# khiner/MeshEditor

Hardware: AMD Instinct MI355X
Metric: eigenpairs/sec (K/M assembly + 50-mode solve, 100k-tet mesh) (higher is better)
Workload: dtype f64; 1 GPU; cube_s100k: Kuhn mesh 105456 tets / 446631 DOF, NumModes=50 NumFemModes=65, P=10 excitation points, one mesh per GPU; eigenpairs_per_mesh=65, kept_modes_per_mesh=50, parallelism=mesh-per-gpu x1

## Files before the change

mesheditor_amd/csrc/lab/mh_lab.hip:

```cpp
#include "../mh_common.h"
#include "modalhip_lab.h"

#include <algorithm>

void mh_elementwise_apply(mh_context *ctx, const mh_system *sys, double sigma, const double *x, double *y, uint32_t w);

namespace {
constexpr int TB = 256;
__global__ void k_lab_ref_to_panel(const double *__restrict__ x, const uint32_t *__restrict__ perm, uint32_t nnodes, uint32_t width, double *__restrict__ panel) {
    const size_t i = size_t(blockIdx.x) * blockDim.x + threadIdx.x;
    if (i >= size_t(nnodes) * 3 * width) return;
    const uint32_t c = uint32_t(i % width), comp = uint32_t((i / width) % 3), node = uint32_t(i / (size_t(3) * width));
    panel[i] = x[size_t(c) * (size_t(3) * nnodes) + size_t(3) * perm[node] + comp];
}
__global__ void k_lab_panel_to_ref(const double *__restrict__ panel, const uint32_t *__restrict__ perm, uint32_t nnodes, uint32_t width, double *__restrict__ y) {
    const size_t i = size_t(blockIdx.x) * blockDim.x + threadIdx.x;
    if (i >= size_t(nnodes) * 3 * width) return;
    const uint32_t c = uint32_t(i % width), comp = uint32_t((i / width) % 3), node = uint32_t(i / (size_t(3) * width));
    y[size_t(c) * (size_t(3) * nnodes) + size_t(3) * perm[node] + comp] = panel[i];
}
}

namespace {
typedef float f4_stream __attribute__((ext_vector_type(4)));
// ... 417 lines not shown
            const std::vector<uint32_t> h = ps.nodes.to_host();
            for (size_t i = 0; i < h.size(); ++i) nodes[i] = node_ref[h[i]];
        }
        if (weight && ps.n_patches) ps.weight.download(weight, ps.n_patches);
        if (inv64 && ps.n_patches) ps.inv64.download(inv64, ps.inv64.count);
        if (cluster_row && ps.n_clusters) {
            const std::vector<uint32_t> h = ps.cluster_row.to_host();
            for (size_t i = 0; i < h.size(); ++i) cluster_row[i] = 3 * node_ref[h[i] / 3] + h[i] % 3;
        }
        if (cluster_ptr && ps.n_clusters) std::copy(ps.h_cluster_ptr.begin(), ps.h_cluster_ptr.end(), cluster_ptr);
        if (cinv64 && ps.n_clusters) ps.cinv64.download(cinv64, ps.cinv64.count);
        return MH_OK;
    } catch (const std::exception &e) { return mh_guard(ctx, e); }
}

int mhl_context_potrf_inverse(mh_context *ctx, uint32_t w, const double *a, const double *dscale, double *l, double *linv, int *info2) {
    if (!ctx || !a || !dscale || !l || !linv || !info2 || w < 1 || w > 128) return MH_EINVAL;
    try {
        HIP_CHECK(hipSetDevice(ctx->device));
        MhSharedPhase not_during_a_factorisation(ctx->device);
        DevArray<double> da(ctx, size_t(w) * w), dd(ctx, w), dl(ctx, size_t(w) * w);
        DevArray<int> info(ctx, 2);
        da.upload(a, size_t(w) * w);
        dd.upload(dscale, w);
        mh_potrf_small_inverse(ctx, da, w, info, dd, dl);
        da.download(l, size_t(w) * w);
        dl.download(linv, size_t(w) * w);
        info.download(info2, 2);
        return MH_OK;
    } catch (const std::exception &e) { return mh_guard(ctx, e); }
}

int mhl_context_spd_inverse(mh_context *ctx, uint32_t w, const double *a, double *out, uint32_t reps, double *avg_ms) {
    if (!ctx || !a || !out || w < 1 || w > 128) return MH_EINVAL;
    try {
        HIP_CHECK(hipSetDevice(ctx->device));
        MhSharedPhase not_during_a_factorisation(ctx->device);
        DevArray<double> da(ctx, size_t(w) * w), dout(ctx, size_t(w) * w);
        DevArray<int> info(ctx, 1);
        info.zero();
        da.upload(a, size_t(w) * w);
        hipEvent_t e0, e1;
        HIP_CHECK(hipEventCreate(&e0));
        HIP_CHECK(hipEventCreate(&e1));
        float total = 0;
        for (uint32_t r = 0; r < std::max(1u, reps); ++r) {
            HIP_CHECK(hipEventRecord(e0, ctx->stream));
            mh_spd_inverse_small(ctx, da, w, w, dout, w, info);
            HIP_CHECK(hipEventRecord(e1, ctx->stream));
            HIP_CHECK(hipEventSynchronize(e1));
            float ms = 0;
            HIP_CHECK(hipEventElapsedTime(&ms, e0, e1));
            total += ms;
        }
        (void)hipEventDestroy(e0);
        (void)hipEventDestroy(e1);
        dout.download(out, size_t(w) * w);
        int hinfo = 0;
        info.download(&hinfo, 1);
        if (avg_ms) *avg_ms = total / std::max(1u, reps);
        return hinfo ? MH_EFACTOR : MH_OK;
    } catch (const std::exception &e) { return mh_guard(ctx, e); }
}

int mhl_context_small_gemm(mh_context *ctx, int ta, int tb, uint32_t M, uint32_t N, uint32_t K, double alpha, const double *a, uint32_t lda, const double *b, uint32_t ldb, double beta,
                           double *c, uint32_t ldc, uint32_t reps, double *avg_ms) {
    if (!ctx || !a || !b || !c || !M || !N || !K || lda < (ta ? K : M) || ldb < (tb ? N : K) || ldc < M) return MH_EINVAL;
    try {
        HIP_CHECK(hipSetDevice(ctx->device));
        MhSharedPhase not_during_a_factorisation(ctx->device);
        const size_t na = size_t(lda) * (ta ? M : K), nb = size_t(ldb) * (tb ? K : N), nc = size_t(ldc) * N;
        DevArray<double> da(ctx, na), db(ctx, nb), dc(ctx, nc), work(ctx, nc);
        da.upload(a, na);
        db.upload(b, nb);
        dc.upload(c, nc);
        hipEvent_t e0, e1;
        HIP_CHECK(hipEventCreate(&e0));
        HIP_CHECK(hipEventCreate(&e1));
        float total = 0;
        for (uint32_t r = 0; r < std::max(1u, reps); ++r) {
            HIP_CHECK(hipMemcpyAsync(work, dc, nc * sizeof(double), hipMemcpyDeviceToDevice, ctx->stream));
// ... 93 lines not shown
```

mesheditor_amd/csrc/mh_common.h:

```cpp
#pragma once
#include "../../include/modalhip.h"

#include <hip/hip_runtime.h>
#include <rocblas/rocblas.h>
#include <rocsolver/rocsolver.h>

#include <algorithm>
#include <cstdarg>
#include <cstdio>
#include <cstdlib>
#include <cstring>
#include <iterator>
#include <limits>
#include <map>
#include <mutex>
#include <stdexcept>
#include <string>
#include <vector>

struct MhError : std::runtime_error {
    int code;
    MhError(int c, const std::string &m) : std::runtime_error(m), code(c) {}
};

// ... 461 lines not shown
uint32_t mh_shift_invert_panel(mh_system *sys, double sigma, const double *b, double *x, uint32_t w, double rel_tol, uint32_t max_iters, double *worst_rel);
struct MhCycleShape {
    int deg2{2}, deg1{5}, gamma{3};
    double ratio{8.0}, ratio1{0.0};
};
void mh_cycle_shape(const mh_system *sys, uint32_t w, MhCycleShape *shape);
double mh_coarse_lift(const mh_system *sys);
void mh_precondition_panel(mh_system *sys, double sigma, int precision, const double *r, double *z, uint32_t w);
uint32_t mh_graph_aggregates(const std::vector<uint32_t> &row_ptr, const std::vector<uint32_t> &col, uint32_t n, uint32_t target, uint32_t max_order, std::vector<uint32_t> &agg_of);
void mh_select_patches(mh_system *sys, float threshold);
void mh_build_patch_inverses(mh_context *ctx, const BsrLevel &lvl, PatchSet &ps);
template<typename T>
void mh_apply_patches(mh_context *ctx, const PatchSet &ps, const T *in, const T *minus, uint32_t w, T coef, T *d, T *x, double *z, uint32_t wz, T *scratch);
void mh_gram(mh_context *ctx, size_t n, const double *x, uint32_t wa, const double *y, uint32_t wb, double *g, uint32_t ld, uint32_t ldy = 0, const uint32_t *ymap = nullptr);
void mh_combine(mh_context *ctx, size_t n, const double *x, uint32_t wx, const double *w, uint32_t ww, const double *p, uint32_t wp, const double *ct, uint32_t nc,
                double *out1, uint32_t n1, double *out2, bool accumulate = false, uint32_t ldx = 0, const uint32_t *xmap = nullptr, uint32_t ld1 = 0,
                const uint32_t *omap = nullptr, uint32_t col_begin = 0, uint32_t col_count = 0);
bool mh_tridiag_lowest_wide(mh_context *ctx, const double *d, const double *e, uint32_t m, uint32_t k, double *w, double *z, uint32_t ldz, double *work, int *info2,
                            double *quality_host);
void mh_apply_q(mh_context *ctx, const double *a, const double *tau, uint32_t m, double *z, uint32_t ldz, uint32_t ncols);
bool mh_tridiag_lowest(mh_context *ctx, const double *d, const double *e, uint32_t m, uint32_t k, double *w, double *z, uint32_t ldz, double *ufac,
                       double *quality, double *lam_scratch);
struct MhRrTrace {
    enum Reduction { GIVEN_IDENTITY = 0, MEASURED_IDENTITY = 1, SERIES = 2, CHOLESKY = 3 };
    enum Solver { SYEVD = 0, SMALL_PARTIAL = 1, SMALL_STEDC = 2, WIDE_PARTIAL = 3, WIDE_STEDC_ORMTR = 4 };
    int reduction{-1};
    double defect{-1};
    int solver{-1};
    double quality{std::numeric_limits<double>::quiet_NaN()};
};
int mh_rr_solve(mh_context *ctx, double *gA, double *gM, uint32_t m, double *evals, double *ework, DevArray<int> &info, uint32_t nwant = 0, bool gm_is_identity = false,
                std::vector<double> *host_evals = nullptr);
void mh_spd_inverse_small(mh_context *ctx, const double *a, uint32_t lda, uint32_t w, double *out, uint32_t ldo, int *info);
void mh_potrf(mh_context *ctx, double *a, uint32_t ld, uint32_t w, int *info);
void mh_potrf_small(mh_context *ctx, double *a, uint32_t w, int *info);
void mh_potrf_small_inverse(mh_context *ctx, double *a, uint32_t w, int *info, const double *dscale, double *linv);
bool mh_sytrd_gave_up(mh_context *ctx);
void mh_sytrd_wide(mh_context *ctx, double *a, uint32_t m, double *d, double *e, double *tau);
void mh_sytrd_small(mh_context *ctx, double *a, uint32_t m, double *d, double *e, double *tau, int variant = -1);
void mh_small_gemm(mh_context *ctx, bool ta, bool tb, uint32_t M, uint32_t N, uint32_t K, double alpha, const double *a, uint32_t lda, const double *b, uint32_t ldb, double beta, double *c,
                   uint32_t ldc);
void mh_short_product(mh_context *ctx, size_t n, const double *a, uint32_t m, const double *ct, uint32_t nc, double *out, double *partial, uint32_t slices);
void mh_pack_stacked(mh_context *ctx, const double *c1, uint32_t r1, const double *c2, uint32_t r2, uint32_t cols, double scale, double *ct);
void mh_pack_coefficients(mh_context *ctx, const double *c1, uint32_t n1, const double *c2, uint32_t n2, uint32_t m, uint32_t ld, double *ct);
void mh_spmm_mapped(mh_context *ctx, const BsrLevel &lvl, const double *vals9, const double *x, double *y, const double *mscal, double *y2, uint32_t w, uint32_t ldy,
                    uint32_t wreal, const uint32_t *omap, const double *res_theta = nullptr, double *res_out = nullptr, double *res_partial = nullptr,
                    const double *res_dinv = nullptr);
bool mh_spmm_f32_cheb_step(mh_context *ctx, const BsrLevel &lvl, const float *d_in, float *d_out, float *r, float *x, const float *dinv, float c1, float c2,
                           uint32_t w);
void mh_spmm_f32(mh_context *ctx, const BsrLevel &lvl, const float *x, float *y, uint32_t w);
void mh_spmm_mixed(mh_context *ctx, const BsrLevel &lvl, const float *x, double *y, uint32_t w);
const uint32_t *mh_identity_map(mh_context *ctx);
void mh_spmm(mh_context *ctx, const BsrLevel &lvl, const double *vals9, const double *x, double *y, const double *mscal, double *y2, uint32_t w);
```

mesheditor_amd/csrc/mh_dense.hip:

```cpp
#include "mh_common.h"

#include <optional>

#include <map>

struct PerDeviceOnce {
    static constexpr int MaxDevices = 64;
    std::once_flag flag[MaxDevices];
    template<typename F> void run(int device, F &&f) { std::call_once(flag[device >= 0 && device < MaxDevices ? device : 0], std::forward<F>(f)); }
};

static bool mh_test_own_gemm() {
    static const bool on = getenv("MH_TEST") && strstr(getenv("MH_TEST"), "own_gemm");
    return on;
}
namespace {
constexpr int KC = 32;

typedef double double4_t __attribute__((ext_vector_type(4)));

__host__ __device__ inline int pad_pitch(int w) {
    int p = ((w + 15) / 16) * 16;
    if ((p % 32) != 16) p += 16;
    return p;
// ... 2121 lines not shown
    const double *ap = A + (a_ok ? ia : 0) * sai + k_lane * sak, *bp = B + (b_ok ? jb : 0) * sbj + k_lane * sbk;
    double4_t acc = {0, 0, 0, 0};
    int k = 0;
    for (; k + 32 <= K; k += 32) {
        double af[8], bf[8];
#pragma unroll
        for (int u = 0; u < 8; ++u) af[u] = ap[(k + 4 * u) * sak], bf[u] = bp[(k + 4 * u) * sbk];
#pragma unroll
        for (int u = 0; u < 8; ++u) acc = __builtin_amdgcn_mfma_f64_16x16x4f64(a_ok ? af[u] : 0.0, b_ok ? bf[u] : 0.0, acc, 0, 0, 0);
    }
    for (; k < K; k += 4) {
        const bool k_ok = k + k_lane < K;
        const double av = a_ok && k_ok ? ap[k * sak] : 0.0, bv = b_ok && k_ok ? bp[k * sbk] : 0.0;
        acc = __builtin_amdgcn_mfma_f64_16x16x4f64(av, bv, acc, 0, 0, 0);
    }
    if (!b_ok) return;
#pragma unroll
    for (int reg = 0; reg < 4; ++reg) {
        const int row = i0 + k_lane + 4 * reg;
        if (row >= M) continue;
        double *c = C + size_t(jb) * ldc + row;
        *c = beta == 0.0 ? alpha * acc[reg] : alpha * acc[reg] + beta * *c;
    }
}
}

void mh_small_gemm(mh_context *ctx, bool ta, bool tb, uint32_t M, uint32_t N, uint32_t K, double alpha, const double *a, uint32_t lda, const double *b, uint32_t ldb, double beta, double *c,
                   uint32_t ldc) {
    if (!M || !N) return;
    const dim3 grid(div_up(M, 32), div_up(N, 32));
    k_small_gemm<<<grid, 256, 0, ctx->stream>>>(int(M), int(N), int(K), alpha, a, ta ? long(lda) : 1L, ta ? 1L : long(lda), b, tb ? long(ldb) : 1L, tb ? 1L : long(ldb), beta, c, int(ldc));
    KERNEL_CHECK();
}
```

mesheditor_amd/csrc/mh_eigs.hip:

```cpp
#include "mh_common.h"

#include <algorithm>
#include <cmath>
#include <memory>
#include <condition_variable>
#include <mutex>
#include <numeric>
#include <optional>
#include <type_traits>

__global__ void k_shift_values(const double *kval, const double *mval, size_t nblocks, double sigma, double *aval);
__global__ void k_diag_inverse(const uint32_t *row_ptr, const uint32_t *col, const double *aval, uint32_t nnodes, double *dinv);
__global__ void k_coarse_matrix(const uint32_t *row_ptr, const uint32_t *col, const double *aval, const double *tmat, const uint32_t *agg_of, const uint32_t *agg_ptr,
                                const uint32_t *agg_nodes, uint32_t nagg, double *a0);
__global__ void k_fix_coarse_diag(double *a0, uint32_t n0, double rel);

namespace {
constexpr int TB = 256;

std::mutex g_solve_mutex;
struct Switches {
    bool verbose = getenv("MH_VERBOSE") != nullptr;
    bool fp32_prec = !(getenv("MH_PRECOND_FP64") && atoi(getenv("MH_PRECOND_FP64")) != 0);
    int deg2 = 0, deg1 = 0, gamma = 0;
// ... 658 lines not shown
    HIP_CHECK(hipMemcpyAsync(saved.get(), gA, size_t(m) * m * sizeof(double), hipMemcpyDeviceToDevice, ctx->stream));
    mh_sytrd_wide(ctx, gA, m, evals, ework, tau);
    int gave_up = 0;
    HIP_CHECK(hipMemcpyAsync(&gave_up, ctx->sytrd_flag, sizeof(int), hipMemcpyDeviceToHost, ctx->stream));
    HIP_CHECK(hipStreamSynchronize(ctx->stream));
    if (sytrd_gave_up(ctx, gave_up, gA, saved, m)) return std::nullopt;
    if (nwant && nwant < m && nwant <= 256 && !switches().no_tridiag_wide) {
        DevArray<double> work(ctx, size_t(5) * nwant * m + size_t(2) * nwant * nwant + 8), lam(ctx, nwant);
        double quality = 1.0;
        if (mh_tridiag_lowest_wide(ctx, evals, ework, m, nwant, lam, z, m, work, info, &quality)) {
            if (switches().verbose) fprintf(stderr, "[rr] tridiagonal m %u lowest %u (wide): residual / ||T|| %.2e\n", m, nwant, quality);
            if (ctx->rr_trace) ctx->rr_trace->quality = quality;
            if (accept_partial(ctx, quality, evals, lam, nwant)) {
                if (ctx->rr_trace) ctx->rr_trace->solver = MhRrTrace::WIDE_PARTIAL;
                mh_apply_q(ctx, gA, tau, m, z, m, nwant);
                rr_selfcheck(ctx, saved.get(), m, z, m, evals, nwant);
                HIP_CHECK(hipMemcpyAsync(gA, z.get(), size_t(m) * nwant * sizeof(double), hipMemcpyDeviceToDevice, ctx->stream));
                HIP_CHECK(hipStreamSynchronize(ctx->stream));
                return 0;
            }
        }
    }
    ROCBLAS_CHECK(rocsolver_dstedc(ctx->blas, rocblas_evect_tridiagonal, m, evals, ework, z, m, info));
    if (const int hinfo = host_info(info)) return hinfo;
    ROCBLAS_CHECK(rocsolver_dormtr(ctx->blas, rocblas_side_left, rocblas_fill_lower, rocblas_operation_none, m, m, gA, m, tau, z, m));
    if (ctx->rr_trace) ctx->rr_trace->solver = MhRrTrace::WIDE_STEDC_ORMTR;
    HIP_CHECK(hipMemcpyAsync(gA, z.get(), size_t(m) * m * sizeof(double), hipMemcpyDeviceToDevice, ctx->stream));
    HIP_CHECK(hipStreamSynchronize(ctx->stream));
    return 0;
}

}

int mh_rr_solve(mh_context *ctx, double *gA, double *gM, uint32_t m, double *evals, double *ework, DevArray<int> &info, uint32_t nwant, bool gm_is_identity,
                std::vector<double> *host_evals) {
    const double one = 1, zero = 0;
    k_symmetrize_lower<<<grid1(size_t(m) * m), TB, 0, ctx->stream>>>(gA, m, m);
    KERNEL_CHECK();
    bool identity = gm_is_identity, series = false;
    if (!identity) {
        static_assert(sizeof(unsigned long long) == sizeof(double), "defect word");
        unsigned long long *defect = reinterpret_cast<unsigned long long *>(ework);
        HIP_CHECK(hipMemsetAsync(defect, 0, sizeof(unsigned long long), ctx->stream));
        k_identity_defect<<<grid1(size_t(m) * m), TB, 0, ctx->stream>>>(gM, m, defect);
        KERNEL_CHECK();
        unsigned long long bits = 0;
        HIP_CHECK(hipMemcpyAsync(&bits, defect, sizeof(bits), hipMemcpyDeviceToHost, ctx->stream));
        HIP_CHECK(hipStreamSynchronize(ctx->stream));
        double d;
        memcpy(&d, &bits, sizeof(d));
        identity = d < 1e-11;
        if (switches().verbose) fprintf(stderr, "[rr] m %u identity defect %.2e\n", m, d);
        series = !identity && d < 1e-7;
        if (ctx->rr_trace) ctx->rr_trace->defect = d;
    }
    if (ctx->rr_trace) ctx->rr_trace->reduction = gm_is_identity ? MhRrTrace::GIVEN_IDENTITY : identity ? MhRrTrace::MEASURED_IDENTITY : series ? MhRrTrace::SERIES : MhRrTrace::CHOLESKY;
    DevArray<double> sroot, stmp;
    if (series) {
        sroot.reset(ctx, size_t(m) * m);
        stmp.reset(ctx, size_t(m) * m * 2);
        double *e = stmp.get(), *e2 = stmp.get() + size_t(m) * m;
        k_defect_matrix<<<grid1(size_t(m) * m), TB, 0, ctx->stream>>>(gM, m, e);
        KERNEL_CHECK();
        small_dgemm(ctx, rocblas_operation_none, rocblas_operation_none, m, m, m, &one, e, m, e, m, &zero, e2, m);
        k_inverse_sqrt_series<<<grid1(size_t(m) * m), TB, 0, ctx->stream>>>(e, e2, m, sroot);
        KERNEL_CHECK();
// ... 315 lines not shown
    {
        const uint32_t nb = 128;
        DevArray<double> &cblk = sys->coarse_ws[0], &rblk = sys->coarse_ws[1], &pnext = sys->coarse_ws[4];
        DevArray<double> *pinv2[2] = {&sys->coarse_ws[2], &sys->coarse_ws[3]};
        cblk.reset(ctx, n0 * nb);
        rblk.reset(ctx, n0 * nb);
        pinv2[0]->reset(ctx, size_t(nb) * nb);
        pinv2[1]->reset(ctx, size_t(nb) * nb);
        pnext.reset(ctx, size_t(nb) * nb);
        info.zero();
        const bool side = ctx->aux_stream_ready();
        struct StreamGuard {
            mh_context *c;
            hipStream_t s;
            bool swapped{false};
            ~StreamGuard() {
                if (c->stream != s) {
                    c->stream = s;
                    if (swapped) std::swap(c->blas, c->blas_aux);
                    (void)hipStreamSynchronize(c->aux_stream);
                    if (c->aux2_stream) (void)hipStreamSynchronize(c->aux2_stream);
                }
            }
        } guard{ctx, main_stream};
        hipEvent_t forked = nullptr;
        if (side) {
            HIP_CHECK(hipEventCreateWithFlags(&forked, hipEventDisableTiming));
            HIP_CHECK(hipEventRecord(forked, main_stream));
            HIP_CHECK(hipStreamWaitEvent(ctx->aux_stream, forked, 0));
            ctx->stream = ctx->aux_stream;
            std::swap(ctx->blas, ctx->blas_aux);
            guard.swapped = true;
        }
        const size_t steps_total = div_up(n0, size_t(nb));
        const bool ahead = side && ctx->aux2_stream_ready(2 * steps_total);
        hipEvent_t *ev_piv = ctx->ahead_ev.data(), *ev_inv = ctx->ahead_ev.data() + steps_total;
        const double one = 1, zero = 0, mone = -1;
        const rocblas_int ld = rocblas_int(n0);
        double *a = sys->a0.get();
        uint32_t step = 0;
        for (size_t k0 = 0; k0 < n0; k0 += nb, ++step) {
            const rocblas_int w = rocblas_int(std::min<size_t>(nb, n0 - k0));
            double *pinv = pinv2[step & 1]->get();
            if (step == 0 || !ahead) mh_spd_inverse_small(ctx, a + k0 * n0 + k0, uint32_t(n0), uint32_t(w), pinv, uint32_t(w), info);
            else HIP_CHECK(hipStreamWaitEvent(ctx->stream, ev_inv[step], 0));
            HIP_CHECK(hipMemcpyAsync(cblk, a + k0 * n0, n0 * size_t(w) * sizeof(double), hipMemcpyDeviceToDevice, ctx->stream));
            ROCBLAS_CHECK(rocblas_dgemm(ctx->blas, rocblas_operation_none, rocblas_operation_none, w, ld, w, &one, pinv, w, a + k0, ld, &zero, rblk, w));
            const size_t k1 = k0 + nb;
            if (ahead && k1 < n0) {
                const uint32_t wn = uint32_t(std::min<size_t>(nb, n0 - k1));
                HIP_CHECK(hipMemcpy2DAsync(pnext.get(), size_t(wn) * sizeof(double), a + k1 * n0 + k1, n0 * sizeof(double), size_t(wn) * sizeof(double), wn, hipMemcpyDeviceToDevice, ctx->stream));
                mh_small_gemm(ctx, false, false, wn, wn, uint32_t(w), -1.0, cblk.get() + k1, uint32_t(n0), rblk.get() + k1 * size_t(w), uint32_t(w), 1.0, pnext.get(), wn);
                HIP_CHECK(hipEventRecord(ev_piv[step], ctx->stream));
                HIP_CHECK(hipStreamWaitEvent(ctx->aux2_stream, ev_piv[step], 0));
                hipStream_t elimination = ctx->stream;
                ctx->stream = ctx->aux2_stream;
                try {
                    mh_spd_inverse_small(ctx, pnext.get(), wn, wn, pinv2[(step + 1) & 1]->get(), wn, info);
                } catch (...) {
                    ctx->stream = elimination;
                    throw;
                }
                ctx->stream = elimination;
                HIP_CHECK(hipEventRecord(ev_inv[step + 1], ctx->aux2_stream));
            }
            ROCBLAS_CHECK(rocblas_dgemm(ctx->blas, rocblas_operation_none, rocblas_operation_none, ld, ld, w, &mone, cblk, ld, rblk, w, &one, a, ld));
            HIP_CHECK(hipMemcpy2DAsync(a + k0, n0 * sizeof(double), rblk.get(), size_t(w) * sizeof(double), size_t(w) * sizeof(double), n0, hipMemcpyDeviceToDevice, ctx->stream));
            ROCBLAS_CHECK(rocblas_dgemm(ctx->blas, rocblas_operation_none, rocblas_operation_none, ld, w, w, &mone, cblk, ld, pinv, w, &zero, a + k0 * n0, ld));
            HIP_CHECK(hipMemcpy2DAsync(a + k0 * n0 + k0, n0 * sizeof(double), pinv, size_t(w) * sizeof(double), size_t(w) * sizeof(double), size_t(w), hipMemcpyDeviceToDevice, ctx->stream));
        }
        k_symmetrize_lower<<<grid1(n0 * n0), TB, 0, ctx->stream>>>(sys->a0, uint32_t(n0), uint32_t(n0));
        KERNEL_CHECK();
        if (side) {
            ctx->stream = main_stream;
            std::swap(ctx->blas, ctx->blas_aux);
        }
        if (!sys->coarse_done) HIP_CHECK(hipEventCreateWithFlags(&sys->coarse_done, hipEventDisableTiming));
        HIP_CHECK(hipEventRecord(sys->coarse_done, side ? ctx->aux_stream : main_stream));
        sys->coarse_pending = true;
        smoother_setup();
        if (side) (void)hipEventDestroy(forked);
    }
    sys->sigma_built = sigma;
    sys->hierarchy_ready = true;
    if (!defer) {
        mh_finish_hierarchy(sys);
        HIP_CHECK(hipStreamSynchronize(ctx->stream));
    }
}

namespace {
__global__ void k_last_columns_to_panel(const double *__restrict__ z, size_t n, uint32_t ncols, const double *__restrict__ scale, double *__restrict__ x) {
    const size_t i = size_t(blockIdx.x) * blockDim.x + threadIdx.x;
    if (i >= n * ncols) return;
    const uint32_t j = uint32_t(i % ncols);
    x[i] = scale[j] * z[(n - 1 - j) * n + i / ncols];
}

void dense_eigs(mh_system *sys, uint32_t nev, double sigma, double *eigenvalues, bool inverse = false) {
    mh_context *ctx = sys->ctx;
    const size_t n = size_t(3) * sys->n_nodes;
    auto &lvl = sys->L2;
    DevArray<double> a(ctx, n * n), m(ctx, n * n), d(ctx, n), e(ctx, n);
    DevArray<int> info(ctx, 1);
    a.zero();
// ... 971 lines not shown
```

mesheditor_amd/csrc/mh_patch.hip:

```cpp
#include "mh_common.h"

namespace {
constexpr int TB = 256;
struct PerDeviceOnce {
    std::mutex m;
    bool done[64] = {};
    template<typename F> void run(int device, F &&f) {
        std::lock_guard<std::mutex> l(m);
        if (!done[unsigned(device) % 64]) f(), done[unsigned(device) % 64] = true;
    }
};

__global__ void k_element_quality(const double *__restrict__ pts, const uint32_t *__restrict__ elem_ref, uint32_t stride, uint32_t nt, float *__restrict__ q, float threshold,
                                  uint32_t *__restrict__ summary) {
    const uint32_t el_raw = blockIdx.x * blockDim.x + threadIdx.x;
    const bool valid = el_raw < nt;
    const uint32_t el = valid ? el_raw : nt - 1;
    double v[4][3];
    for (int a = 0; a < 4; ++a)
        for (int d = 0; d < 3; ++d) v[a][d] = pts[3 * size_t(elem_ref[size_t(el) * stride + a]) + d];
    const double bx = v[1][0] - v[0][0], by = v[1][1] - v[0][1], bz = v[1][2] - v[0][2];
    const double cx = v[2][0] - v[0][0], cy = v[2][1] - v[0][1], cz = v[2][2] - v[0][2];
    const double dx = v[3][0] - v[0][0], dy = v[3][1] - v[0][1], dz = v[3][2] - v[0][2];
    const double vol = fabs(dx * (by * cz - cy * bz) + dy * (bz * cx - cz * bx) + dz * (bx * cy - cx * by)) / 6;
// ... 227 lines not shown
        if (r >= N) continue;
#pragma unroll
        for (int j = 0; j < 4; ++j) {
            const uint32_t cc = col0 + tx * 4 + j;
            if (cc < w) y[size_t(r0 + r) * w + cc] = acc[i][j];
        }
    }
}

template<typename T>
__global__ void k_cluster_scatter(const T *__restrict__ y, uint32_t w, const uint32_t *__restrict__ crow, uint32_t nrows, T coef, T *__restrict__ d, T *__restrict__ x, double *__restrict__ z,
                                  uint32_t wz, int slices) {
    const size_t i = size_t(blockIdx.x) * blockDim.x + threadIdx.x;
    if (i >= size_t(nrows) * w) return;
    const uint32_t c = uint32_t(i % w);
    const size_t row = crow[i / w];
    T sum = 0;
    for (int q = 0; q < slices; ++q) sum += y[size_t(q) * nrows * w + i];
    const T s = coef * sum;
    if (d) d[row * w + c] += s;
    if (x) x[row * w + c] += s;
    if (z && c < wz) z[row * wz + c] += double(s);
}

__global__ void k_f64_to_f32(const double *__restrict__ in, float *__restrict__ out, size_t count) {
    const size_t i = size_t(blockIdx.x) * blockDim.x + threadIdx.x;
    if (i < count) out[i] = float(in[i]);
}
__global__ void k_copy_block(const double *__restrict__ in, uint32_t ldi, double *__restrict__ out, uint32_t ldo, uint32_t rows, uint32_t cols) {
    const size_t i = size_t(blockIdx.x) * blockDim.x + threadIdx.x;
    if (i >= size_t(rows) * cols) return;
    const size_t c = i / rows, r = i % rows;
    out[c * ldo + r] = in[c * ldi + r];
}
__global__ void k_symmetrize(double *__restrict__ a, uint32_t n) {
    const size_t i = size_t(blockIdx.x) * blockDim.x + threadIdx.x;
    if (i >= size_t(n) * n) return;
    const size_t r = i / n, c = i % n;
    if (c < r) {
        const double v = 0.5 * (a[r * n + c] + a[c * n + r]);
        a[r * n + c] = v;
        a[c * n + r] = v;
    }
}
}

void mh_select_patches(mh_system *sys, float threshold) {
    mh_context *ctx = sys->ctx;
    hipStream_t st = ctx->stream;
    const uint32_t nt = sys->kept_tets;
    sys->patches2 = PatchSet{};
    sys->patches1 = PatchSet{};
    sys->patches2.npe = 10;
    sys->patches1.npe = 4;
    if (!(threshold > 0) || nt == 0) return;
    DevArray<float> q(ctx, nt);
    DevArray<uint32_t> summary(ctx, 2);
    const uint32_t init[2] = {0u, 0x7f7fffffu};
    summary.upload(init, 2);
    k_element_quality<<<div_up(nt, TB), TB, 0, st>>>(sys->points, sys->elem_nodes_ref, 10, nt, q, threshold, summary);
    KERNEL_CHECK();
    uint32_t hs[2];
    summary.download(hs, 2);
    memcpy(&sys->worst_quality, &hs[1], sizeof(float));
    if (hs[0] == 0) return;
    const std::vector<float> hq = q.to_host();
    std::vector<uint32_t> bad;
    for (uint32_t e = 0; e < nt; ++e)
        if (hq[e] < threshold) bad.push_back(e);
    std::vector<uint32_t> en(size_t(nt) * 10), ep(size_t(nt) * 4);
    HIP_CHECK(hipMemcpyAsync(en.data(), sys->elem_nodes.get(), en.size() * sizeof(uint32_t), hipMemcpyDeviceToHost, st));
    HIP_CHECK(hipMemcpyAsync(ep.data(), sys->elem_p1.get(), ep.size() * sizeof(uint32_t), hipMemcpyDeviceToHost, st));
    HIP_CHECK(hipStreamSynchronize(st));
    constexpr double overlap_exponent = -0.35;
    static const int cluster_switch = getenv("MH_CLUSTERS") ? atoi(getenv("MH_CLUSTERS")) : -1;
    const bool flat_cells = sys->worst_quality < 1e-4f;
// ... 112 lines not shown
            ps.tile_cluster.reset(ctx, tile_cluster.size());
            ps.tile_row0.reset(ctx, tile_row0.size());
            ps.cluster_row.upload(crow.data(), crow.size());
            ps.cluster_ptr.upload(cptr.data(), cptr.size());
            ps.cluster_inv_ptr.upload(iptr.data(), iptr.size());
            ps.tile_cluster.upload(tile_cluster.data(), tile_cluster.size());
            ps.tile_row0.upload(tile_row0.data(), tile_row0.size());
            ps.cinv64.reset(ctx, iptr.back());
            ps.cinv32.reset(ctx, iptr.back());
        }
        HIP_CHECK(hipStreamSynchronize(st));
    };
    const auto regroup = [&](bool clusters) {
        single.clear();
        multi.clear();
        std::vector<int32_t> slot(bad.size(), -1);
        for (uint32_t k = 0; k < bad.size(); ++k) {
            if (!clusters || comp_size[comp[k]] == 1) { single.push_back(k); continue; }
            if (slot[comp[k]] < 0) slot[comp[k]] = int32_t(multi.size()), multi.emplace_back();
            multi[size_t(slot[comp[k]])].push_back(k);
        }
    };
    regroup(use_clusters);
    if (getenv("MH_DEBUG_PATCH")) fprintf(stderr, "[patch] single %zu multi %zu\n", single.size(), multi.size());
    fill(sys->patches2, en, 10, sys->n_nodes);
    if (getenv("MH_DEBUG_PATCH")) fprintf(stderr, "[patch] P2 filled: clusters %u rows %u largest %u\n", sys->patches2.n_clusters, sys->patches2.cluster_rows, sys->patches2.largest_cluster);
    if (cluster_switch == 2) regroup(true);
    fill(sys->patches1, ep, 4, sys->n_points);
    if (getenv("MH_DEBUG_PATCH")) fprintf(stderr, "[patch] P1 filled: clusters %u rows %u largest %u\n", sys->patches1.n_clusters, sys->patches1.cluster_rows, sys->patches1.largest_cluster);
}

static int spd_inverse_in_place(mh_context *ctx, double *a, uint32_t n) {
    const uint32_t nb = 128;
    DevArray<double> cblk(ctx, size_t(n) * nb), rblk(ctx, size_t(n) * nb), pinv(ctx, size_t(nb) * nb);
    DevArray<int> info(ctx, 1);
    info.zero();
    const double one = 1, zero = 0, mone = -1;
    const rocblas_int ld = rocblas_int(n);
    for (uint32_t k0 = 0; k0 < n; k0 += nb) {
        const rocblas_int w = rocblas_int(std::min(nb, n - k0));
        mh_spd_inverse_small(ctx, a + size_t(k0) * n + k0, n, uint32_t(w), pinv, uint32_t(w), info);
        HIP_CHECK(hipMemcpyAsync(cblk, a + size_t(k0) * n, size_t(n) * size_t(w) * sizeof(double), hipMemcpyDeviceToDevice, ctx->stream));
        ROCBLAS_CHECK(rocblas_dgemm(ctx->blas, rocblas_operation_none, rocblas_operation_none, w, ld, w, &one, pinv, w, a + k0, ld, &zero, rblk, w));
        ROCBLAS_CHECK(rocblas_dgemm(ctx->blas, rocblas_operation_none, rocblas_operation_none, ld, ld, w, &mone, cblk, ld, rblk, w, &one, a, ld));
        HIP_CHECK(hipMemcpy2DAsync(a + k0, size_t(n) * sizeof(double), rblk.get(), size_t(w) * sizeof(double), size_t(w) * sizeof(double), n, hipMemcpyDeviceToDevice, ctx->stream));
        ROCBLAS_CHECK(rocblas_dgemm(ctx->blas, rocblas_operation_none, rocblas_operation_none, ld, w, w, &mone, cblk, ld, pinv, w, &zero, a + size_t(k0) * n, ld));
        HIP_CHECK(hipMemcpy2DAsync(a + size_t(k0) * n + k0, size_t(n) * sizeof(double), pinv.get(), size_t(w) * sizeof(double), size_t(w) * sizeof(double), size_t(w), hipMemcpyDeviceToDevice, ctx->stream));
    }
    k_symmetrize<<<div_up(size_t(n) * n, TB), TB, 0, ctx->stream>>>(a, n);
    KERNEL_CHECK();
    int h = 0;
    info.download(&h, 1);
    return h;
}

void mh_build_patch_inverses(mh_context *ctx, const BsrLevel &lvl, PatchSet &ps) {
    if (!ps.any()) return;
    ps.dropped.reset(ctx, 2);
    ps.dropped.zero();
    if (ps.n_patches) {
        const size_t n = size_t(3) * ps.npe;
        ps.inv64.reset(ctx, size_t(ps.n_patches) * n * n);
        ps.inv32.reset(ctx, size_t(ps.n_patches) * n * n);
        if (ps.npe == 10) k_patch_inverse<10><<<ps.n_patches, 64, 0, ctx->stream>>>(lvl.row_ptr, lvl.col, lvl.aval, ps.nodes, ps.weight, ps.n_patches, ps.inv64, ps.inv32, ps.dropped);
        else k_patch_inverse<4><<<ps.n_patches, 64, 0, ctx->stream>>>(lvl.row_ptr, lvl.col, lvl.aval, ps.nodes, ps.weight, ps.n_patches, ps.inv64, ps.inv32, ps.dropped);
        KERNEL_CHECK();
    }
    if (!ps.n_clusters) return;
    k_cluster_block<<<dim3(ps.n_clusters, 64), TB, 0, ctx->stream>>>(lvl.row_ptr, lvl.col, lvl.aval, ps.cluster_row, ps.cluster_ptr, ps.cluster_inv_ptr, ps.cinv64);
    KERNEL_CHECK();
    std::vector<uint32_t> small, large;
    for (uint32_t c = 0; c < ps.n_clusters; ++c) (ps.h_cluster_ptr[c + 1] - ps.h_cluster_ptr[c] <= 128 ? small : large).push_back(c);
    if (!small.empty()) {
        DevArray<uint32_t> list(ctx, small.size());
        list.upload(small.data(), small.size());
        static PerDeviceOnce attr;
        attr.run(ctx->device, [] { HIP_CHECK(hipFuncSetAttribute(reinterpret_cast<const void *>(&k_cluster_inverse_lds), hipFuncAttributeMaxDynamicSharedMemorySize, 140 * 1024)); });
        k_cluster_inverse_lds<<<uint32_t(small.size()), 128, size_t(128) * 129 * sizeof(double), ctx->stream>>>(list, ps.cluster_ptr, ps.cluster_inv_ptr, ps.cinv64, ps.dropped);
        KERNEL_CHECK();
        HIP_CHECK(hipStreamSynchronize(ctx->stream));
    }
    if (!large.empty()) {
        std::vector<uint64_t> iptr(ps.n_clusters + 1);
// ... 51 lines not shown
```

Baseline: 612.3 eigenpairs/s.

## Replace rocBLAS Gauss-Jordan SPD inverse with custom MFMA panel/update kernels

Replaces the blocked Gauss-Jordan SPD inverse, which used per-step rocBLAS dgemms plus device copies, with two custom MFMA f64 kernels. A panel kernel fuses the block copy, the row-block product and the column update. A symmetric update kernel touches only the off-diagonal block pairs of one triangle. The shared routine keeps the look-ahead pivot inversion on the aux stream and is now used by both the coarse solve and the patch inverses. The aim is to cut launch count, extra copies and redundant full-matrix GEMM work, at the cost of hand-tuned kernels that may be slower than rocBLAS on some shapes.

```diff
diff --git a/mesheditor_amd/csrc/lab/mh_lab.hip b/mesheditor_amd/csrc/lab/mh_lab.hip
--- a/mesheditor_amd/csrc/lab/mh_lab.hip
+++ b/mesheditor_amd/csrc/lab/mh_lab.hip
@@ -473,11 +473,15 @@
 }
 
 int mhl_context_spd_inverse(mh_context *ctx, uint32_t w, const double *a, double *out, uint32_t reps, double *avg_ms) {
-    if (!ctx || !a || !out || w < 1 || w > 128) return MH_EINVAL;
-    try {
-        HIP_CHECK(hipSetDevice(ctx->device));
-        MhSharedPhase not_during_a_factorisation(ctx->device);
+    if (!ctx || !a || !out || w < 1 || w > 16384) return MH_EINVAL;
+    try {
+        HIP_CHECK(hipSetDevice(ctx->device));
+        MhSharedPhase not_during_a_factorisation(ctx->device);
+        const bool blocked = w > 128;
+        const size_t nb = 128;
         DevArray<double> da(ctx, size_t(w) * w), dout(ctx, size_t(w) * w);
+        DevArray<double> cblk(ctx, blocked ? w * nb : 0), rblk(ctx, blocked ? w * nb : 0), pinv0(ctx, blocked ? nb * nb : 0), pinv1(ctx, blocked ? nb * nb : 0);
+        const MhSpdInverseWork ws{cblk.get(), rblk.get(), {pinv0.get(), pinv1.get()}, nullptr};
         DevArray<int> info(ctx, 1);
         info.zero();
         da.upload(a, size_t(w) * w);
@@ -486,8 +490,10 @@
         HIP_CHECK(hipEventCreate(&e1));
         float total = 0;
         for (uint32_t r = 0; r < std::max(1u, reps); ++r) {
+            if (blocked) HIP_CHECK(hipMemcpyAsync(dout, da, size_t(w) * w * sizeof(double), hipMemcpyDeviceToDevice, ctx->stream));
             HIP_CHECK(hipEventRecord(e0, ctx->stream));
-            mh_spd_inverse_small(ctx, da, w, w, dout, w, info);
+            if (blocked) mh_spd_inverse_blocked(ctx, dout, w, ws, info, false);
+            else mh_spd_inverse_small(ctx, da, w, w, dout, w, info);
             HIP_CHECK(hipEventRecord(e1, ctx->stream));
             HIP_CHECK(hipEventSynchronize(e1));
             float ms = 0;
diff --git a/mesheditor_amd/csrc/mh_common.h b/mesheditor_amd/csrc/mh_common.h
--- a/mesheditor_amd/csrc/mh_common.h
+++ b/mesheditor_amd/csrc/mh_common.h
@@ -517,6 +517,11 @@
 int mh_rr_solve(mh_context *ctx, double *gA, double *gM, uint32_t m, double *evals, double *ework, DevArray<int> &info, uint32_t nwant = 0, bool gm_is_identity = false,
                 std::vector<double> *host_evals = nullptr);
 void mh_spd_inverse_small(mh_context *ctx, const double *a, uint32_t lda, uint32_t w, double *out, uint32_t ldo, int *info);
+struct MhSpdInverseWork {
+    double *cblk, *rblk, *pinv[2], *pnext;
+};
+void mh_spd_inverse_blocked(mh_context *ctx, double *a, uint32_t n, const MhSpdInverseWork &ws, int *info, bool ahead);
+void mh_symmetrize_lower(mh_context *ctx, double *a, uint32_t n);
 void mh_potrf(mh_context *ctx, double *a, uint32_t ld, uint32_t w, int *info);
 void mh_potrf_small(mh_context *ctx, double *a, uint32_t w, int *info);
 void mh_potrf_small_inverse(mh_context *ctx, double *a, uint32_t w, int *info, const double *dscale, double *linv);
diff --git a/mesheditor_amd/csrc/mh_dense.hip b/mesheditor_amd/csrc/mh_dense.hip
--- a/mesheditor_amd/csrc/mh_dense.hip
+++ b/mesheditor_amd/csrc/mh_dense.hip
@@ -2177,3 +2177,171 @@
     k_small_gemm<<<grid, 256, 0, ctx->stream>>>(int(M), int(N), int(K), alpha, a, ta ? long(lda) : 1L, ta ? 1L : long(lda), b, tb ? long(ldb) : 1L, tb ? 1L : long(ldb), beta, c, int(ldc));
     KERNEL_CHECK();
 }
+
+namespace {
+constexpr int GJ_NB = 128;
+
+__global__ void __launch_bounds__(256) k_gj_panel(double *__restrict__ a, int n, int k0, int w, const double *__restrict__ pinv, double *__restrict__ cblk, double *__restrict__ rt) {
+    const int lane = threadIdx.x & 63, wave = threadIdx.x >> 6, l15 = lane & 15, kl = lane >> 4;
+    const int bk = k0 / GJ_NB, b = blockIdx.y, j0 = b * GJ_NB + int(blockIdx.x) * 16;
+    if (j0 >= n) return;
+    const size_t ld = size_t(n);
+    if (b == bk) {
+        const int c = j0 - k0 + (threadIdx.x >> 4);
+        if (c < w)
+            for (int r = l15; r < w; r += 16) a[size_t(k0 + c) * ld + k0 + r] = pinv[size_t(c) * w + r];
+        return;
+    }
+    const bool below = b > bk;
+    const int j = j0 + l15, jc = min(j, n - 1);
+    const double *xp = below ? a + size_t(k0) * ld + jc : a + size_t(jc) * ld + k0;
+    const size_t xs = below ? ld : 1;
+    const int rf = wave * 32;
+    const int r0 = min(rf + l15, w - 1), r1 = min(rf + 16 + l15, w - 1);
+    const double *pp0 = pinv + r0, *pp1 = pinv + r1;
+    const double *pt0 = pinv + size_t(r0) * w, *pt1 = pinv + size_t(r1) * w;
+    const bool f0 = rf < w, f1 = rf + 16 < w;
+    double4_t acc0 = {0, 0, 0, 0}, acc1 = {0, 0, 0, 0}, col0 = {0, 0, 0, 0}, col1 = {0, 0, 0, 0};
+    const double sign = below ? 1.0 : -1.0;
+    for (int ks = 0; ks < w; ks += 4) {
+        const int c = ks + kl, cc = min(c, w - 1);
+        const bool ok = c < w;
+        double x = xp[size_t(cc) * xs];
+        x = ok ? x : 0.0;
+        if (((ks >> 2) & 3) == wave && ok && j < n) cblk[size_t(c) * ld + j] = sign * x;
+        if (f0) {
+            const double p = pp0[size_t(cc) * w];
+            acc0 = __builtin_amdgcn_mfma_f64_16x16x4f64(ok ? p : 0.0, x, acc0, 0, 0, 0);
+            if (below) col0 = __builtin_amdgcn_mfma_f64_16x16x4f64(ok ? pt0[cc] : 0.0, x, col0, 0, 0, 0);
+        }
+        if (f1) {
+            const double p = pp1[size_t(cc) * w];
+            acc1 = __builtin_amdgcn_mfma_f64_16x16x4f64(ok ? p : 0.0, x, acc1, 0, 0, 0);
+            if (below) col1 = __builtin_amdgcn_mfma_f64_16x16x4f64(ok ? pt1[cc] : 0.0, x, col1, 0, 0, 0);
+        }
+    }
+    mh_lds_writes_landed();
+    __syncthreads();
+    if (j >= n) return;
+#pragma unroll
+    for (int f = 0; f < 2; ++f) {
+        if (!(f ? f1 : f0)) continue;
+#pragma unroll
+        for (int reg = 0; reg < 4; ++reg) {
+            const int r = rf + 16 * f + 4 * reg + kl;
+            if (r >= w) continue;
+            const double v = f ? acc1[reg] : acc0[reg];
+            rt[size_t(r) * ld + j] = v;
+            if (below) a[size_t(k0 + r) * ld + j] = -(f ? col1[reg] : col0[reg]);
+            else a[size_t(j) * ld + k0 + r] = v;
+        }
+    }
+}
+
+constexpr int GJ_TI = 4, GJ_TJ = 2;
+__global__ void __launch_bounds__(256) k_gj_update(double *__restrict__ a, int n, int bk, int w, const double *__restrict__ cblk, const double *__restrict__ rt) {
+    const int lane = threadIdx.x & 63, wave = threadIdx.x >> 6, l15 = lane & 15, kl = lane >> 4;
+    const int p = int(blockIdx.x) >> 1, half = int(blockIdx.x) & 1;
+    int ci = int((sqrtf(8.0f * float(p) + 1.0f) - 1.0f) * 0.5f);
+    while ((ci + 1) * (ci + 2) / 2 <= p) ++ci;
+    while (ci * (ci + 1) / 2 > p) --ci;
+    const int cj = p - ci * (ci + 1) / 2;
+    const int bi = ci + (ci >= bk ? 1 : 0), bj = cj + (cj >= bk ? 1 : 0);
+    const int i0 = bi * GJ_NB + (wave & 1) * 64, j0 = bj * GJ_NB + half * 64 + (wave >> 1) * 32;
+    if (i0 >= n || j0 >= n) return;
+    const size_t ld = size_t(n);
+    const double *cp[GJ_TI], *rp[GJ_TJ];
+#pragma unroll
+    for (int t = 0; t < GJ_TI; ++t) cp[t] = cblk + min(i0 + 16 * t + l15, n - 1);
+#pragma unroll
+    for (int t = 0; t < GJ_TJ; ++t) rp[t] = rt + min(j0 + 16 * t + l15, n - 1);
+    double4_t acc[GJ_TJ][GJ_TI];
+#pragma unroll
+    for (int tj = 0; tj < GJ_TJ; ++tj)
+#pragma unroll
+        for (int ti = 0; ti < GJ_TI; ++ti)
+#pragma unroll
+            for (int reg = 0; reg < 4; ++reg) acc[tj][ti][reg] = a[size_t(min(j0 + 16 * tj + 4 * reg + kl, n - 1)) * ld + min(i0 + 16 * ti + l15, n - 1)];
+    int ks = 0;
+    for (; ks + 16 <= w; ks += 16) {
+        double cf[4][GJ_TI], rf[4][GJ_TJ];
+#pragma unroll
+        for (int u = 0; u < 4; ++u) {
+            const size_t off = size_t(ks + 4 * u + kl) * ld;
+#pragma unroll
+            for (int t = 0; t < GJ_TI; ++t) cf[u][t] = cp[t][off];
+#pragma unroll
+            for (int t = 0; t < GJ_TJ; ++t) rf[u][t] = -rp[t][off];
+        }
+#pragma unroll
+        for (int u = 0; u < 4; ++u)
+#pragma unroll
+            for (int tj = 0; tj < GJ_TJ; ++tj)
+#pragma unroll
+                for (int ti = 0; ti < GJ_TI; ++ti) acc[tj][ti] = __builtin_amdgcn_mfma_f64_16x16x4f64(rf[u][tj], cf[u][ti], acc[tj][ti], 0, 0, 0);
+    }
+    for (; ks < w; ks += 4) {
+        const int c = ks + kl;
+        const bool ok = c < w;
+        const size_t off = size_t(min(c, w - 1)) * ld;
+        double cf[GJ_TI], rf[GJ_TJ];
+#pragma unroll
+        for (int t = 0; t < GJ_TI; ++t) cf[t] = ok ? cp[t][off] : 0.0;
+#pragma unroll
+        for (int t = 0; t < GJ_TJ; ++t) rf[t] = ok ? -rp[t][off] : 0.0;
+#pragma unroll
+        for (int tj = 0; tj < GJ_TJ; ++tj)
+#pragma unroll
+            for (int ti = 0; ti < GJ_TI; ++ti) acc[tj][ti] = __builtin_amdgcn_mfma_f64_16x16x4f64(rf[tj], cf[ti], acc[tj][ti], 0, 0, 0);
+    }
+#pragma unroll
+    for (int tj = 0; tj < GJ_TJ; ++tj)
+#pragma unroll
+        for (int ti = 0; ti < GJ_TI; ++ti)
+#pragma unroll
+            for (int reg = 0; reg < 4; ++reg) {
+                const int i = i0 + 16 * ti + l15, j = j0 + 16 * tj + 4 * reg + kl;
+                if (i < n && j < n) a[size_t(j) * ld + i] = acc[tj][ti][reg];
+            }
+}
+}
+
+void mh_spd_inverse_blocked(mh_context *ctx, double *a, uint32_t n, const MhSpdInverseWork &ws, int *info, bool ahead) {
+    if (!n) return;
+    const uint32_t nb = GJ_NB, steps_total = div_up(n, nb);
+    if (ahead && (!ctx->aux2_stream || ctx->ahead_ev.size() < 2 * size_t(steps_total))) mh_throw(MH_EINVAL, "spd_inverse_blocked: look-ahead without its stream and events");
+    hipEvent_t *ev_piv = ctx->ahead_ev.data(), *ev_inv = ctx->ahead_ev.data() + steps_total;
+    uint32_t step = 0;
+    for (uint32_t k0 = 0; k0 < n; k0 += nb, ++step) {
+        const uint32_t w = std::min(nb, n - k0);
+        double *pinv = ws.pinv[step & 1];
+        if (step == 0 || !ahead) mh_spd_inverse_small(ctx, a + size_t(k0) * n + k0, n, w, pinv, w, info);
+        else HIP_CHECK(hipStreamWaitEvent(ctx->stream, ev_inv[step], 0));
+        k_gj_panel<<<dim3(nb / 16, steps_total), 256, 0, ctx->stream>>>(a, int(n), int(k0), int(w), pinv, ws.cblk, ws.rblk);
+        KERNEL_CHECK();
+        const uint32_t k1 = k0 + nb;
+        if (ahead && k1 < n) {
+            const uint32_t wn = std::min(nb, n - k1);
+            HIP_CHECK(hipMemcpy2DAsync(ws.pnext, size_t(wn) * sizeof(double), a + size_t(k1) * n + k1, size_t(n) * sizeof(double), size_t(wn) * sizeof(double), wn, hipMemcpyDeviceToDevice, ctx->stream));
+            mh_small_gemm(ctx, false, true, wn, wn, w, -1.0, ws.cblk + k1, n, ws.rblk + k1, n, 1.0, ws.pnext, wn);
+            HIP_CHECK(hipEventRecord(ev_piv[step], ctx->stream));
+            HIP_CHECK(hipStreamWaitEvent(ctx->aux2_stream, ev_piv[step], 0));
+            hipStream_t elimination = ctx->stream;
+            ctx->stream = ctx->aux2_stream;
+            try {
+                mh_spd_inverse_small(ctx, ws.pnext, wn, wn, ws.pinv[(step + 1) & 1], wn, info);
+            } catch (...) {
+                ctx->stream = elimination;
+                throw;
+            }
+            ctx->stream = elimination;
+            HIP_CHECK(hipEventRecord(ev_inv[step + 1], ctx->aux2_stream));
+        }
+        if (steps_total > 1) {
+            const uint32_t others = steps_total - 1;
+            k_gj_update<<<others * (others + 1), 256, 0, ctx->stream>>>(a, int(n), int(step), int(w), ws.cblk, ws.rblk);
+            KERNEL_CHECK();
+        }
+    }
+    mh_symmetrize_lower(ctx, a, n);
+}
diff --git a/mesheditor_amd/csrc/mh_eigs.hip b/mesheditor_amd/csrc/mh_eigs.hip
--- a/mesheditor_amd/csrc/mh_eigs.hip
+++ b/mesheditor_amd/csrc/mh_eigs.hip
@@ -714,6 +714,11 @@
 
 }
 
+void mh_symmetrize_lower(mh_context *ctx, double *a, uint32_t n) {
+    k_symmetrize_lower<<<grid1(size_t(n) * n), TB, 0, ctx->stream>>>(a, n, n);
+    KERNEL_CHECK();
+}
+
 int mh_rr_solve(mh_context *ctx, double *gA, double *gM, uint32_t m, double *evals, double *ework, DevArray<int> &info, uint32_t nwant, bool gm_is_identity,
                 std::vector<double> *host_evals) {
     const double one = 1, zero = 0;
@@ -1095,45 +1100,9 @@
             std::swap(ctx->blas, ctx->blas_aux);
             guard.swapped = true;
         }
-        const size_t steps_total = div_up(n0, size_t(nb));
-        const bool ahead = side && ctx->aux2_stream_ready(2 * steps_total);
-        hipEvent_t *ev_piv = ctx->ahead_ev.data(), *ev_inv = ctx->ahead_ev.data() + steps_total;
-        const double one = 1, zero = 0, mone = -1;
-        const rocblas_int ld = rocblas_int(n0);
-        double *a = sys->a0.get();
-        uint32_t step = 0;
-        for (size_t k0 = 0; k0 < n0; k0 += nb, ++step) {
-            const rocblas_int w = rocblas_int(std::min<size_t>(nb, n0 - k0));
-            double *pinv = pinv2[step & 1]->get();
-            if (step == 0 || !ahead) mh_spd_inverse_small(ctx, a + k0 * n0 + k0, uint32_t(n0), uint32_t(w), pinv, uint32_t(w), info);
-            else HIP_CHECK(hipStreamWaitEvent(ctx->stream, ev_inv[step], 0));
-            HIP_CHECK(hipMemcpyAsync(cblk, a + k0 * n0, n0 * size_t(w) * sizeof(double), hipMemcpyDeviceToDevice, ctx->stream));
-            ROCBLAS_CHECK(rocblas_dgemm(ctx->blas, rocblas_operation_none, rocblas_operation_none, w, ld, w, &one, pinv, w, a + k0, ld, &zero, rblk, w));
-            const size_t k1 = k0 + nb;
-            if (ahead && k1 < n0) {
-                const uint32_t wn = uint32_t(std::min<size_t>(nb, n0 - k1));
-                HIP_CHECK(hipMemcpy2DAsync(pnext.get(), size_t(wn) * sizeof(double), a + k1 * n0 + k1, n0 * sizeof(double), size_t(wn) * sizeof(double), wn, hipMemcpyDeviceToDevice, ctx->stream));
-                mh_small_gemm(ctx, false, false, wn, wn, uint32_t(w), -1.0, cblk.get() + k1, uint32_t(n0), rblk.get() + k1 * size_t(w), uint32_t(w), 1.0, pnext.get(), wn);
-                HIP_CHECK(hipEventRecord(ev_piv[step], ctx->stream));
-                HIP_CHECK(hipStreamWaitEvent(ctx->aux2_stream, ev_piv[step], 0));
-                hipStream_t elimination = ctx->stream;
-                ctx->stream = ctx->aux2_stream;
-                try {
-                    mh_spd_inverse_small(ctx, pnext.get(), wn, wn, pinv2[(step + 1) & 1]->get(), wn, info);
-                } catch (...) {
-                    ctx->stream = elimination;
-                    throw;
-                }
-                ctx->stream = elimination;
-                HIP_CHECK(hipEventRecord(ev_inv[step + 1], ctx->aux2_stream));
-            }
-            ROCBLAS_CHECK(rocblas_dgemm(ctx->blas, rocblas_operation_none, rocblas_operation_none, ld, ld, w, &mone, cblk, ld, rblk, w, &one, a, ld));
-            HIP_CHECK(hipMemcpy2DAsync(a + k0, n0 * sizeof(double), rblk.get(), size_t(w) * sizeof(double), size_t(w) * sizeof(double), n0, hipMemcpyDeviceToDevice, ctx->stream));
-            ROCBLAS_CHECK(rocblas_dgemm(ctx->blas, rocblas_operation_none, rocblas_operation_none, ld, w, w, &mone, cblk, ld, pinv, w, &zero, a + k0 * n0, ld));
-            HIP_CHECK(hipMemcpy2DAsync(a + k0 * n0 + k0, n0 * sizeof(double), pinv, size_t(w) * sizeof(double), size_t(w) * sizeof(double), size_t(w), hipMemcpyDeviceToDevice, ctx->stream));
-        }
-        k_symmetrize_lower<<<grid1(n0 * n0), TB, 0, ctx->stream>>>(sys->a0, uint32_t(n0), uint32_t(n0));
-        KERNEL_CHECK();
+        const bool ahead = side && ctx->aux2_stream_ready(2 * size_t(div_up(n0, size_t(nb))));
+        const MhSpdInverseWork ws{cblk.get(), rblk.get(), {pinv2[0]->get(), pinv2[1]->get()}, pnext.get()};
+        mh_spd_inverse_blocked(ctx, sys->a0.get(), uint32_t(n0), ws, info, ahead);
         if (side) {
             ctx->stream = main_stream;
             std::swap(ctx->blas, ctx->blas_aux);
diff --git a/mesheditor_amd/csrc/mh_patch.hip b/mesheditor_amd/csrc/mh_patch.hip
--- a/mesheditor_amd/csrc/mh_patch.hip
+++ b/mesheditor_amd/csrc/mh_patch.hip
@@ -283,16 +283,6 @@
     if (i >= size_t(rows) * cols) return;
     const size_t c = i / rows, r = i % rows;
     out[c * ldo + r] = in[c * ldi + r];
-}
-__global__ void k_symmetrize(double *__restrict__ a, uint32_t n) {
-    const size_t i = size_t(blockIdx.x) * blockDim.x + threadIdx.x;
-    if (i >= size_t(n) * n) return;
-    const size_t r = i / n, c = i % n;
-    if (c < r) {
-        const double v = 0.5 * (a[r * n + c] + a[c * n + r]);
-        a[r * n + c] = v;
-        a[c * n + r] = v;
-    }
 }
 }
 
@@ -471,23 +461,10 @@
 
 static int spd_inverse_in_place(mh_context *ctx, double *a, uint32_t n) {
     const uint32_t nb = 128;
-    DevArray<double> cblk(ctx, size_t(n) * nb), rblk(ctx, size_t(n) * nb), pinv(ctx, size_t(nb) * nb);
+    DevArray<double> cblk(ctx, size_t(n) * nb), rblk(ctx, size_t(n) * nb), pinv0(ctx, size_t(nb) * nb), pinv1(ctx, size_t(nb) * nb);
     DevArray<int> info(ctx, 1);
     info.zero();
-    const double one = 1, zero = 0, mone = -1;
-    const rocblas_int ld = rocblas_int(n);
-    for (uint32_t k0 = 0; k0 < n; k0 += nb) {
-        const rocblas_int w = rocblas_int(std::min(nb, n - k0));
-        mh_spd_inverse_small(ctx, a + size_t(k0) * n + k0, n, uint32_t(w), pinv, uint32_t(w), info);
-        HIP_CHECK(hipMemcpyAsync(cblk, a + size_t(k0) * n, size_t(n) * size_t(w) * sizeof(double), hipMemcpyDeviceToDevice, ctx->stream));
-        ROCBLAS_CHECK(rocblas_dgemm(ctx->blas, rocblas_operation_none, rocblas_operation_none, w, ld, w, &one, pinv, w, a + k0, ld, &zero, rblk, w));
-        ROCBLAS_CHECK(rocblas_dgemm(ctx->blas, rocblas_operation_none, rocblas_operation_none, ld, ld, w, &mone, cblk, ld, rblk, w, &one, a, ld));
-        HIP_CHECK(hipMemcpy2DAsync(a + k0, size_t(n) * sizeof(double), rblk.get(), size_t(w) * sizeof(double), size_t(w) * sizeof(double), n, hipMemcpyDeviceToDevice, ctx->stream));
-        ROCBLAS_CHECK(rocblas_dgemm(ctx->blas, rocblas_operation_none, rocblas_operation_none, ld, w, w, &mone, cblk, ld, pinv, w, &zero, a + size_t(k0) * n, ld));
-        HIP_CHECK(hipMemcpy2DAsync(a + size_t(k0) * n + k0, size_t(n) * sizeof(double), pinv.get(), size_t(w) * sizeof(double), size_t(w) * sizeof(double), size_t(w), hipMemcpyDeviceToDevice, ctx->stream));
-    }
-    k_symmetrize<<<div_up(size_t(n) * n, TB), TB, 0, ctx->stream>>>(a, n);
-    KERNEL_CHECK();
+    mh_spd_inverse_blocked(ctx, a, n, MhSpdInverseWork{cblk.get(), rblk.get(), {pinv0.get(), pinv1.get()}, nullptr}, info, false);
     int h = 0;
     info.download(&h, 1);
     return h;
```

New measurement: 613.9 eigenpairs/s, median of 2. About the same (+0.3%).
